# zhaozijie2022/LocoTouch

Hardware: AMD Instinct MI355X
Metric: env-steps/sec (whole node), TransportTeacher 4096 envs/GPU (higher is better)
Workload: dtype f32

## Files before the change

include/lt_env.h:

```cpp
#ifndef LT_ENV_H
#define LT_ENV_H

#include <stddef.h>
#include <stdint.h>

#ifdef __cplusplus
extern "C" {
#endif

#define LT_ABI_VERSION 21

#define LT_OK 0
#define LT_EINVAL (-22)
#define LT_ENOMEM (-12)
#define LT_EFAULT (-14)
#define LT_EHIP (-5)

#define LT_TASK_LOCOMOTION 0
#define LT_TASK_TRANSPORT_TEACHER 1
#define LT_TACTILE_ROWS 17
#define LT_TACTILE_COLS 13
#define LT_TACTILE_DIM 442
#define LT_TACTILE_WIDE_DIM 884
#define LT_TACTILE_BINARY 0
// ... 325 lines not shown
  LT_PRIM_TRUNK = 0, LT_PRIM_BACK_MID = 1, LT_PRIM_PLATE = 2, LT_PRIM_RAIL_LEFT = 3, LT_PRIM_RAIL_RIGHT = 4,
  LT_PRIM_HIP = 5,
  LT_PRIM_THIGH = 9,
  LT_PRIM_CALF = 13,
  LT_PRIM_FOOT = 17,
  LT_PRIM_OBJECT = 21, LT_PRIM_GROUND = 22, LT_RENDER_NUM_PRIMS = 23
};
#define LT_RENDER_MAX_SIZE 8192
#define LT_RENDER_FAR 1000
#define LT_RENDER_DEPTH_MISS 1000000
#define LT_RENDER_VIEWS_PER_LAUNCH 32
typedef struct lt_render_view {
  int32_t env_id;
  int32_t origin;
  float eye[3];
  float lookat[3];
  float fov_y_deg;
} lt_render_view;
typedef struct lt_render_desc {
  int32_t width, height;
  int32_t flags;
  float light_dir[3];
} lt_render_desc;
int lt_env_render(lt_env* env, const lt_render_desc* desc, const lt_render_view* views, int nviews, uint32_t* rgba, float* depth,
                  int32_t* ids, float* poses, void* stream);

const char* lt_env_kernel_name(int which);
enum lt_mlp_mode { LT_MLP_MODE_FORWARD = 0, LT_MLP_MODE_POLICY = 1, LT_MLP_MODE_BACKWARD = 2 };
const char* lt_mlp_kernel_name(const lt_mlp_desc* d0, const lt_mlp_desc* d1_or_null, int64_t m, int mode);

#include "lt_obs_norm.h"
#include "lt_student.h"
#include "lt_collect.h"

#ifdef __cplusplus
}
#endif
#endif
```

locotouch_amd/_abi.py:

```python
from __future__ import annotations

import ctypes
import os
import re

_HERE = os.path.dirname(os.path.abspath(__file__))
REPO = os.path.dirname(_HERE)
HEADER = os.path.join(REPO, "include", "lt_env.h")
OBS_NORM_HEADER = os.path.join(REPO, "include", "lt_obs_norm.h")
STUDENT_HEADER = os.path.join(REPO, "include", "lt_student.h")
COLLECT_HEADER = os.path.join(REPO, "include", "lt_collect.h")
LIB_PATH = os.environ.get("LOCOTOUCH_AMD_LIB", os.path.join(_HERE, "_lib", "liblocotouch_env.so"))

_SCALARS = {"int": ctypes.c_int, "int32_t": ctypes.c_int32, "int64_t": ctypes.c_int64, "uint8_t": ctypes.c_uint8,
            "uint32_t": ctypes.c_uint32, "uint64_t": ctypes.c_uint64, "size_t": ctypes.c_size_t, "float": ctypes.c_float,
            "double": ctypes.c_double}
_DECL = re.compile(r"(?:const\s+)?(\w+)\s*((?:\*\s*(?:const\b\s*)?)*)(\w*)\s*((?:\[[^\]]*\]\s*)*)")


def _ctype(decl, structs, opaque, consts, typed, param):
    m = _DECL.fullmatch(decl.strip())
    if not m:
        return None
    base, stars, name, dims = m.groups()
    depth = stars.count("*")
    try:
        dims = [sum(int(t) if t.strip().isdigit() else consts[t.strip()] for t in d.split("+")) for d in re.findall(r"\[([^\]]*)\]", dims)]
    except KeyError:
        return None
    if param and dims:
        depth, dims = depth + 1, dims[1:]
    t = structs.get(base) or _SCALARS.get(base)
    if (t is None and base not in opaque and base not in ("void", "char")) or depth > 2 or (param and dims):
        return None
    if depth == 0 and t is None:
        return None
    if depth == 1 and base == "char":
        t = ctypes.c_char_p
    elif depth == 1:
        t = ctypes.POINTER(t) if t is not None and (typed or base in structs or base == "size_t") else ctypes.c_void_p
    elif depth == 2:
        t = ctypes.POINTER(ctypes.POINTER(t) if typed and t is not None else ctypes.c_void_p)
    for d in reversed(dims):
        t = t * d
# ... 56 lines not shown
        return {name: py(getattr(self, name)) for name, *_ in self._fields_ if not name.startswith("_")}


CONSTS, STRUCTS, SIGNATURES = parse_header(open(HEADER).read(), bases={"lt_cfg": _CfgMethods})
globals().update(CONSTS)
LtCfg, LtView, LtMlpDesc = STRUCTS["lt_cfg"], STRUCTS["lt_view"], STRUCTS["lt_mlp_desc"]
LtRenderView, LtRenderDesc = STRUCTS["lt_render_view"], STRUCTS["lt_render_desc"]
EXPORTS = list(SIGNATURES)
OBS_NORM_SIGNATURES = parse_header(open(OBS_NORM_HEADER).read())[2]
if any(r is not ctypes.c_int for r, _ in OBS_NORM_SIGNATURES.values()) or set(OBS_NORM_SIGNATURES) & set(EXPORTS):
    raise ImportError("include/lt_obs_norm.h: every entry point returns a status and none repeats one of lt_env.h")

VALUE_QUERIES = frozenset({
    "lt_abi_version", "lt_cfg_sizeof", "lt_cfg_num_presets", "lt_cfg_preset_id", "lt_cfg_obs_dim", "lt_cfg_tactile_dim", "lt_last_error",
    "lt_wgrad_splits", "lt_wgrad_ws_floats", "lt_elu_backward_bias_ws_floats", "lt_head_wgrad_ws_floats", "lt_adam_clip_step_ws_floats",
    "lt_elu_backward_bias_nblk", "lt_head_wgrad_nblk", "lt_mlp_backward_blocks", "lt_env_kernel_name", "lt_mlp_kernel_name"})
if not VALUE_QUERIES <= set(EXPORTS) or any(SIGNATURES[n][0] is not ctypes.c_int for n in set(EXPORTS) - VALUE_QUERIES):
    raise ImportError("_abi.VALUE_QUERIES does not match include/lt_env.h: a query it names is gone, or a new entry point returns no status")

STUDENT_CONSTS, _student_structs, STUDENT_SIGNATURES = parse_header(open(STUDENT_HEADER).read(), structs=STRUCTS)
globals().update(STUDENT_CONSTS)
LtStudentDesc, LtStudentParams = _student_structs["lt_student_desc"], _student_structs["lt_student_params"]
STUDENT_VALUE_QUERIES = frozenset({"lt_student_step_launches"})
if (not STUDENT_VALUE_QUERIES <= set(STUDENT_SIGNATURES) or any(r is not ctypes.c_int for r, _ in STUDENT_SIGNATURES.values())
        or set(STUDENT_SIGNATURES) & (set(EXPORTS) | set(OBS_NORM_SIGNATURES))):
    raise ImportError("_abi.STUDENT_VALUE_QUERIES does not match include/lt_student.h, or an entry point there returns no int or repeats "
                      "one of another header")

COLLECT_SIGNATURES = parse_header(open(COLLECT_HEADER).read())[2]
if (any(r is not ctypes.c_int for r, _ in COLLECT_SIGNATURES.values())
        or set(COLLECT_SIGNATURES) & (set(EXPORTS) | set(OBS_NORM_SIGNATURES) | set(STUDENT_SIGNATURES))):
    raise ImportError("include/lt_collect.h: every entry point returns a status and none repeats one of another header")

_lib = None
_calls: dict = {}


def load() -> ctypes.CDLL:
    global _lib
    if _lib is not None:
        return _lib
    if not os.path.exists(LIB_PATH):
        raise ImportError(f"{LIB_PATH} is missing: run `python -c 'import __graft_entry__ as g; g.build()'` "
                          "(the HIP extension is mandatory, there is no CPU fallback)")
    lib = ctypes.CDLL(LIB_PATH)
    for name, (restype, argtypes) in {**SIGNATURES, **OBS_NORM_SIGNATURES, **STUDENT_SIGNATURES, **COLLECT_SIGNATURES}.items():
        fn = getattr(lib, name)
        fn.restype, fn.argtypes = restype, argtypes
        if name not in VALUE_QUERIES and name not in STUDENT_VALUE_QUERIES:
            _calls[name] = (fn, [ptr if t is ctypes.c_void_p else _ref if issubclass(t, ctypes._Pointer) and issubclass(t._type_, ctypes.Structure)
                                 else None for t in argtypes])
    if lib.lt_cfg_sizeof() != ctypes.sizeof(LtCfg):
        raise ImportError(f"lt_cfg ABI mismatch: C {lib.lt_cfg_sizeof()} vs ctypes {ctypes.sizeof(LtCfg)}")
    if lib.lt_abi_version() != CONSTS["LT_ABI_VERSION"]:
        raise ImportError("lt_env.h / liblocotouch_env.so ABI version mismatch")
    _lib = lib
    return lib


def ptr(x):
    if x is None or isinstance(x, int):
        return ctypes.c_void_p(x or None)
    data_ptr = getattr(x, "data_ptr", None)
    return ctypes.c_void_p(data_ptr()) if data_ptr else x


def _ref(x):
    return ctypes.byref(x) if isinstance(x, ctypes.Structure) else x


def stream(device=None) -> ctypes.c_void_p:
    import torch

    return ctypes.c_void_p(torch.cuda.current_stream(device).cuda_stream)


def ptr_array(tensors):
    return (ctypes.c_void_p * max(1, len(tensors)))(*[None if t is None else t.data_ptr() for t in tensors])

# ... 50 lines not shown
```

locotouch_amd/csrc/lt_ppo.hip:

```cpp
#include <hip/hip_runtime.h>
#include <math.h>
#include <stdint.h>

#include "lt_env.h"
#include "lt_internal.h"

namespace {

constexpr int MAX_A = 16;
constexpr float kHalfLog2Pi = 0.91893853320467274178f;

__global__ __launch_bounds__(256) void lt_ppo_loss_kernel(const float* __restrict__ mu, const float* __restrict__ stdp, const float* __restrict__ value,
                                                          const float* __restrict__ actions, const float* __restrict__ old_logp,
                                                          const float* __restrict__ adv, const float* __restrict__ returns,
                                                          const float* __restrict__ old_values, const float* __restrict__ old_mu,
                                                          const float* __restrict__ old_sigma, const long long* __restrict__ idx,
                                                          long long M, int A, float clip, float vcoef, int clipped_value,
                                                          float* __restrict__ dmu, float* __restrict__ dvalue, float* __restrict__ acc) {
  const long long row = (long long)blockIdx.x * 256 + threadIdx.x;
  const bool ok = row < M;
  const long long src = (ok && idx) ? idx[row] : row;
  float part[4 + MAX_A];
  float amax_mu = 0.f, amax_v = 0.f;
#pragma unroll
// ... 59 lines not shown
    if (lane == 0) red[wave][i] = v;
  }
#pragma unroll
  for (int off = 32; off > 0; off >>= 1) {
    amax_mu = fmaxf(amax_mu, __shfl_xor(amax_mu, off, 64));
    amax_v = fmaxf(amax_v, __shfl_xor(amax_v, off, 64));
  }
  __shared__ float redm[4][2];
  if (lane == 0) { redm[wave][0] = amax_mu; redm[wave][1] = amax_v; }
  __syncthreads();
  if (threadIdx.x < 4 + A && threadIdx.x != 3) {
    const int i = threadIdx.x;
    atomicAdd(acc + i, red[0][i] + red[1][i] + red[2][i] + red[3][i]);
  } else if (threadIdx.x >= 64 && threadIdx.x < 66) {
    const int j = threadIdx.x - 64;
    atomicMax((unsigned*)acc + 20 + j, __float_as_uint(fmaxf(fmaxf(redm[0][j], redm[1][j]), fmaxf(redm[2][j], redm[3][j]))));
  }
}

__global__ __launch_bounds__(64) void lt_ppo_finalize_kernel(const float* __restrict__ acc, const float* __restrict__ stdp, int A, float inv_m,
                                                             float vcoef, float ecoef, float* __restrict__ out) {
  const int a = threadIdx.x;
  float e = 0.f;
  if (a < A) {
    const float sg = stdp[a];
    e = 0.5f + kHalfLog2Pi + logf(sg);
    out[8 + a] = acc[4 + a] - ecoef / sg;
  }
  for (int off = 32; off > 0; off >>= 1) e += __shfl_xor(e, off, 64);
  if (a == 0) {
    const float surr = acc[0] * inv_m, vl = acc[1] * inv_m;
    out[0] = surr + vcoef * vl - ecoef * e;
    out[1] = surr; out[2] = vl; out[3] = e; out[4] = acc[2] * inv_m;
  }
}

constexpr int EB_ROWS = 48;

__global__ __launch_bounds__(256) void lt_elu_bwd_bias_kernel(const float* da, const float* __restrict__ a, long long M, int N, float alpha,
                                                              float* dz, float* __restrict__ ws, float* __restrict__ amax) {
  const int n4 = N >> 2, lanes = 256 / n4;
  const int c4 = threadIdx.x % n4, rl = threadIdx.x / n4;
  const long long r0 = (long long)blockIdx.x * EB_ROWS;
  float4 sum = {0.f, 0.f, 0.f, 0.f};
  float mx = 0.f;
  if (rl < lanes) {
    for (int r = rl; r < EB_ROWS; r += lanes) {
      const long long row = r0 + r;
      if (row >= M) break;
      const float4 g = ((const float4*)(da + row * N))[c4], y = ((const float4*)(a + row * N))[c4];
      float4 o;
      o.x = g.x * (y.x > 0.f ? 1.f : y.x + alpha);
      o.y = g.y * (y.y > 0.f ? 1.f : y.y + alpha);
      o.z = g.z * (y.z > 0.f ? 1.f : y.z + alpha);
      o.w = g.w * (y.w > 0.f ? 1.f : y.w + alpha);
      ((float4*)(dz + row * N))[c4] = o;
      sum.x += o.x; sum.y += o.y; sum.z += o.z; sum.w += o.w;
      mx = fmaxf(fmaxf(mx, fmaxf(fabsf(o.x), fabsf(o.y))), fmaxf(fabsf(o.z), fabsf(o.w)));
    }
  }
  __shared__ float4 red[256];
  __shared__ float redm[4];
  red[threadIdx.x] = sum;
  if (amax) {
#pragma unroll
    for (int off = 32; off > 0; off >>= 1) mx = fmaxf(mx, __shfl_xor(mx, off, 64));
// ... 76 lines not shown
        s[u].x += v.x; s[u].y += v.y; s[u].z += v.z; s[u].w += v.w;
      }
    }
#pragma unroll
    for (int u = 0; u < 3; ++u) {
      if (b < nblk) {
        const float4 v = at(b);
        s[u].x += v.x; s[u].y += v.y; s[u].z += v.z; s[u].w += v.w;
        b += RL;
      }
    }
  }
  __shared__ float4 red[256];
  red[threadIdx.x] = make_float4((s[0].x + s[1].x) + (s[2].x + s[3].x), (s[0].y + s[1].y) + (s[2].y + s[3].y),
                                 (s[0].z + s[1].z) + (s[2].z + s[3].z), (s[0].w + s[1].w) + (s[2].w + s[3].w));
  __syncthreads();
  if (lane == 0 && e < count) {
    float4 t = red[c];
    for (int l = 1; l < RL; ++l) { const float4 v = red[l * cols + c]; t.x += v.x; t.y += v.y; t.z += v.z; t.w += v.w; }
    const float o[4] = {t.x, t.y, t.z, t.w};
#pragma unroll
    for (int i = 0; i < 4; ++i) {
      const int ei = e + i;
      if (ei >= count) break;
      if (ei < split) J.out0[j][ei] = o[i];
      else if (J.out1[j]) J.out1[j][ei - split] = o[i];
    }
  }
}

constexpr int HW_ROWS = 96, HW_MAX_N = 16;

template <int NN>
__global__ __launch_bounds__(256) void lt_head_wgrad_kernel(const float* __restrict__ dy, const float* __restrict__ x, int x_split, long long M, int n, int k,
                                                            float* __restrict__ ws) {
  const int k4 = k >> 2, lanes = 256 / k4;
  const int c4 = threadIdx.x % k4, rl = threadIdx.x / k4;
  const long long r0 = (long long)blockIdx.x * HW_ROWS;
  float4 acc[NN];
  float accb[NN];
#pragma unroll
  for (int j = 0; j < NN; ++j) { acc[j] = {0.f, 0.f, 0.f, 0.f}; accb[j] = 0.f; }
  if (rl < lanes) {
    for (int r = rl; r < HW_ROWS; r += 4 * lanes) {
      float4 xv[4];
      float d[4][NN];
#pragma unroll
      for (int u = 0; u < 4; ++u) {
        const long long row = r0 + r + u * lanes;
        const bool ok = (r + u * lanes) < HW_ROWS && row < M;
        xv[u] = ok ? ((const float4*)(x + row * k))[c4] : float4{0.f, 0.f, 0.f, 0.f};
        if (x_split) {
          const unsigned w[4] = {__float_as_uint(xv[u].x), __float_as_uint(xv[u].y), __float_as_uint(xv[u].z), __float_as_uint(xv[u].w)};
          float f[4];
#pragma unroll
          for (int i = 0; i < 4; ++i)
            f[i] = (float)__builtin_bit_cast(_Float16, (unsigned short)(w[i] & 0xFFFFu)) + (float)__builtin_bit_cast(_Float16, (unsigned short)(w[i] >> 16)) * (1.f / 64.f);
          xv[u] = float4{f[0], f[1], f[2], f[3]};
        }
#pragma unroll
        for (int j = 0; j < NN; ++j) d[u][j] = (ok && j < n) ? dy[row * n + j] : 0.f;
      }
#pragma unroll
      for (int u = 0; u < 4; ++u)
#pragma unroll
        for (int j = 0; j < NN; ++j) {
          acc[j].x += d[u][j] * xv[u].x; acc[j].y += d[u][j] * xv[u].y; acc[j].z += d[u][j] * xv[u].z; acc[j].w += d[u][j] * xv[u].w;
          accb[j] += d[u][j];
        }
    }
  }
  extern __shared__ float4 red[];
  float* const redb = (float*)(red + (size_t)lanes * NN * k4);
  if (rl < lanes) {
#pragma unroll
    for (int j = 0; j < NN; ++j) red[((size_t)rl * NN + j) * k4 + c4] = acc[j];
    if (c4 == 0)
#pragma unroll
      for (int j = 0; j < NN; ++j) redb[rl * NN + j] = accb[j];
  }
  __syncthreads();
  float* const out = ws + (size_t)blockIdx.x * ((size_t)n * k + HW_MAX_N);
  for (int e = threadIdx.x; e < n * k4; e += 256) {
    const int j = e / k4, c = e - j * k4;
    float4 t = red[(size_t)j * k4 + c];
    for (int l = 1; l < lanes; ++l) {
      const float4 u = red[((size_t)l * NN + j) * k4 + c];
      t.x += u.x; t.y += u.y; t.z += u.z; t.w += u.w;
    }
    ((float4*)(out + (size_t)j * k))[c] = t;
  }
  if (threadIdx.x < n) {
    float t = redb[threadIdx.x];
    for (int l = 1; l < lanes; ++l) t += redb[l * NN + threadIdx.x];
    out[(size_t)n * k + threadIdx.x] = t;
  }
}

__global__ __launch_bounds__(256) void lt_gae_kernel(const float* __restrict__ rewards, const unsigned char* __restrict__ dones,
                                                     const float* __restrict__ values, const float* __restrict__ last_values, float gamma,
                                                     float lam, int T, long long N, float* __restrict__ returns, float* __restrict__ advantages) {
  const long long e = (long long)blockIdx.x * 256 + threadIdx.x;
  if (e >= N) return;
  float next_v = last_values[e], gae = 0.f;
  for (int t = T - 1; t >= 0; --t) {
    const long long o = (long long)t * N + e;
    const float v = values[o], alive = 1.f - (float)dones[o];
    const float delta = rewards[o] + alive * gamma * next_v - v;
    gae = delta + alive * gamma * lam * gae;
    const float ret = gae + v;
    returns[o] = ret;
    advantages[o] = ret - v;
    next_v = v;
  }
}

constexpr int AD_PER_BLOCK = 2048;

__global__ __launch_bounds__(256) void lt_sumsq_kernel(const float* __restrict__ g, long long n, float* __restrict__ ws) {
  const long long base = (long long)blockIdx.x * AD_PER_BLOCK;
  float s = 0.f;
  for (int k = threadIdx.x; k < AD_PER_BLOCK; k += 256) {
    const long long i = base + k;
    if (i < n) s += g[i] * g[i];
  }
  for (int off = 32; off > 0; off >>= 1) s += __shfl_xor(s, off, 64);
  __shared__ float red[4];
  if ((threadIdx.x & 63) == 0) red[threadIdx.x >> 6] = s;
  __syncthreads();
// ... 177 lines not shown
    lt_set_error("lt_adam_clip_step: invalid argument");
    return LT_EINVAL;
  }
  const int nblk = (int)((n + AD_PER_BLOCK - 1) / AD_PER_BLOCK);
  const double bc1 = 1.0 - pow((double)beta1, (double)step), bc2 = 1.0 - pow((double)beta2, (double)step);
  hipLaunchKernelGGL(lt_sumsq_kernel, dim3((unsigned)nblk), dim3(256), 0, (hipStream_t)stream, grads, (long long)n, ws);
  hipLaunchKernelGGL(lt_adam_kernel, dim3((unsigned)nblk), dim3(256), 0, (hipStream_t)stream, params, grads, exp_avg, exp_avg_sq, (long long)n, ws, nblk,
                     max_norm, beta1, beta2, eps, weight_decay, (float)((double)lr / bc1), (float)sqrt(bc2), grad_norm, lr_dev, (float)(1.0 / bc1));
  const hipError_t e = hipGetLastError();
  if (e != hipSuccess) { lt_set_error(hipGetErrorString(e)); return LT_EHIP; }
  return LT_OK;
}

extern "C" int64_t lt_adam_clip_step_ws_floats(int64_t n) { return (n + AD_PER_BLOCK - 1) / AD_PER_BLOCK; }

extern "C" int lt_ppo_loss(const float* mu, const float* stdp, const float* value, const float* actions, const float* old_logp, const float* adv,
                           const float* returns, const float* old_values, const float* old_mu, const float* old_sigma, const int64_t* idx,
                           int64_t M, int A, float clip, float value_loss_coef, float entropy_coef, int use_clipped_value_loss, float* dmu, float* dvalue,
                           float* acc, float* out, void* stream) {
  if (!mu || !stdp || !value || !actions || !old_logp || !adv || !returns || !old_values || !old_mu || !old_sigma || !dmu || !dvalue || !acc ||
      M < 1 || A < 1 || A > MAX_A) {
    lt_set_error("lt_ppo_loss: invalid argument (1 <= num_actions <= 16)");
    return LT_EINVAL;
  }
  hipError_t e = hipMemsetAsync(acc, 0, sizeof(float) * (4 + MAX_A + 4), (hipStream_t)stream);
  if (e != hipSuccess) { lt_set_error(hipGetErrorString(e)); return LT_EHIP; }
  hipLaunchKernelGGL(lt_ppo_loss_kernel, dim3((unsigned)((M + 255) / 256)), dim3(256), 0, (hipStream_t)stream, mu, stdp, value, actions, old_logp, adv,
                     returns, old_values, old_mu, old_sigma, (const long long*)idx, (long long)M, A, clip, value_loss_coef, use_clipped_value_loss, dmu, dvalue, acc);
  if (out) hipLaunchKernelGGL(lt_ppo_finalize_kernel, dim3(1), dim3(64), 0, (hipStream_t)stream, acc, stdp, A, 1.f / (float)M, value_loss_coef, entropy_coef, out);
  e = hipGetLastError();
  if (e != hipSuccess) { lt_set_error(hipGetErrorString(e)); return LT_EHIP; }
  return LT_OK;
}
```

locotouch_amd/rl/mlp.py:

```python
from __future__ import annotations

import ctypes
import os

import torch
import torch.nn as nn

from .. import _abi

USE_FUSED_BACKWARD = os.environ.get("LT_FUSED_BACKWARD", "1") != "0"
_ACT_IDS = {nn.ELU: "LT_ACT_ELU", nn.ReLU: "LT_ACT_RELU", nn.Tanh: "LT_ACT_TANH", nn.Identity: "LT_ACT_NONE"}


def describe(seq: nn.Sequential):
    linears, acts = [], set()
    mods = list(seq)
    for i, m in enumerate(mods):
        if isinstance(m, nn.Linear):
            if m.bias is None or m.weight.dtype != torch.float32:
                return None
            linears.append(m)
        elif type(m) in _ACT_IDS:
            if type(m) is nn.ELU and (m.alpha != 1.0):
                return None
            if i == 0 or not isinstance(mods[i - 1], nn.Linear) or i == len(mods) - 1:
                return None
            acts.add(type(m))
        else:
            return None
    C = _abi.CONSTS
    if not linears or len(linears) > C["LT_MLP_MAX_LAYERS"] or len(acts) > 1:
        return None
    if len(linears) > 1 and len(mods) != 2 * len(linears) - 1:
        return None
    dims = [linears[0].in_features] + [l.out_features for l in linears]
    if dims[0] > C["LT_MLP_MAX_WIDTH"] or any(d > 512 for d in dims[1:]):
        return None
    if any(a.out_features != b.in_features for a, b in zip(linears[:-1], linears[1:])):
        return None
    desc = _abi.LtMlpDesc()
    desc.num_layers = len(linears)
    for i, d in enumerate(dims):
        desc.dims[i] = d
# ... 233 lines not shown
        self.domain_max = None
        return v >= float(_abi.CONSTS["LT_MLP_INPUT_CLAMP"])

    def forward_raw(self, x0: torch.Tensor, x1: torch.Tensor, split: bool | None = None):
        if split is None:
            split = self._fused_backward_possible(x0, x1)
        self.acts_split = bool(split)
        self.pack_training(with_backward=self.acts_split)
        ys, acts = _forward_pair((self.a, self.b), x0, x1, self.acts_split)
        if self.check_domain:
            hidden = [t.view(torch.float16)[:, 0::2] if self.acts_split else t for t in (*acts[0], *acts[1])]
            self._record_domain((x0, x1, *hidden))
        return ys, acts

    def pack_training(self, with_backward: bool) -> None:
        args = []
        for net in (self.a, self.b):
            if with_backward:
                net.alloc_bpacked()
            args += [net.desc, net.weight_ptrs(), net.bias_ptrs(), net.packed, net.bpacked if with_backward else None]
        _abi.call("lt_mlp_pack_training", *args, _abi.stream())
        self._bpacked_fresh = bool(with_backward)

    def split_rows(self, x: torch.Tensor) -> torch.Tensor:
        k = x.shape[1]
        if k % 4:
            xp = torch.zeros(x.shape[0], k + (-k) % 4, device=x.device, dtype=torch.float32)
            xp[:, :k] = x
            x = xp
        out = torch.empty_like(x, dtype=torch.float32)
        _abi.call("lt_split_rows", x, out, x.numel(), _abi.stream())
        return out

    def _fused_backward_possible(self, x0, x1) -> bool:
        from .linear import _head_wgrad_ok

        if not USE_FUSED_BACKWARD:
            return False
        if x0.dtype != torch.float32 or x1.dtype != torch.float32 or not x0.is_contiguous() or not x1.is_contiguous():
            return False
        if self._bwd_shapes_ok is None:
            ok = self.a.backward_ok() and self.b.backward_ok()
            for net in (self.a, self.b):
                dims = [net.desc.dims[i] for i in range(net.desc.num_layers + 1)]
                ok = ok and dims[0] % 2 == 0
                ok = ok and _head_wgrad_ok(torch.empty(0, dims[-1], device=x0.device), torch.empty(0, dims[-2], device=x0.device))
            self._bwd_shapes_ok = bool(ok)
        return self._bwd_shapes_ok

    def _fused_backward_ok(self, x0, x1, dy0, dy1) -> bool:
        return self._fused_backward_possible(x0, x1) and dy0.dtype == torch.float32 and dy1.dtype == torch.float32

    def _backward_fused(self, x0, x1, acts, dy0, dy1, grad_of, sums, x_split_rows=None, after_first=None, dy_amax=None) -> None:
        lib = _abi.load()
        stream = _abi.stream()
        m = x0.shape[0]
        nets, xs = (self.a, self.b), (x0, x1)
        asp = int(self.acts_split)
        xsp = int(x_split_rows is not None)
        if not xsp and any(x.shape[1] % 4 for x in xs):
            x_split_rows, xsp = (self.split_rows(x0), self.split_rows(x1)), 1
        if xsp:
            xs = x_split_rows
        dys = [d if d.is_contiguous() else d.contiguous() for d in (dy0, dy1)]
        dev = x0.device
        if self.sat is None:
            self.sat = torch.zeros(1, device=dev, dtype=torch.float32)
        nblk = lib.lt_mlp_backward_blocks(ctypes.byref(nets[0].desc), ctypes.byref(nets[1].desc), m)
        dzs, amaxs, arrs = [], [], []
        per_net = (SumJobs(), SumJobs()) if after_first is not None else (sums, sums)
        for k, net in enumerate(nets):
            if not self._bpacked_fresh:
                net.pack_backward()
            L = len(net.linears)
            n, kk = dys[k].shape[1], acts[k][L - 2].shape[1]
            ws = torch.empty(lib.lt_head_wgrad_ws_floats(m, n, kk), device=dev, dtype=torch.float32)
            _abi.call("lt_head_wgrad", dys[k], acts[k][L - 2], asp, m, n, kk, None, None, ws, stream)
            per_net[k].add(ws, lib.lt_head_wgrad_nblk(m), n * kk + 16, n * kk + n, n * kk, grad_of[net.linears[L - 1].weight], grad_of[net.linears[L - 1].bias])
            dz = [torch.empty_like(a) for a in acts[k]]
            am = torch.empty(L - 1, nblk, device=dev, dtype=torch.float32)
            dzs.append(dz)
            amaxs.append(am)
            arrs.append((_abi.ptr_array(acts[k]), _abi.ptr_array(dz), _abi.ptr_array([am[l] for l in range(L - 1)])))
        dzsp = int(dy_amax is not None)
        scales = torch.empty(2, device=dev, dtype=torch.float32)
        in_amax = dy_amax if dzsp else (None, None)
        _abi.call("lt_mlp_backward_pair", nets[0].desc, nets[0].bpacked, dys[0], *arrs[0], nets[1].desc, nets[1].bpacked, dys[1], *arrs[1],
                  m, asp, in_amax[0], in_amax[1], dzsp, scales, self.sat, stream)
        for k, net in enumerate(nets):
            for l in range(len(net.linears) - 2, -1, -1):
                inp = acts[k][l - 1] if l > 0 else xs[k]
                dz = dzs[k][l]
                n, kk = dz.shape[1], inp.shape[1]
                sp = lib.lt_wgrad_splits(m, n, kk)
                slabs = torch.empty(sp * n * kk + sp * n, device=dev, dtype=torch.float32)
                dbs = slabs[sp * n * kk:]
                _abi.call("lt_wgrad", dz, dzsp, scales[k:k + 1], inp, asp if l > 0 else xsp, m, n, kk, amaxs[k][l], nblk, slabs, dbs, stream)
                gw = grad_of[net.linears[l].weight]
                if kk != gw.shape[1]:
                    pad = torch.empty(n, kk, device=dev, dtype=torch.float32)
                    per_net[k].add(slabs, sp, n * kk, n * kk, n * kk, pad)
                    per_net[k].after.append((gw, pad[:, :gw.shape[1]]))
                else:
                    per_net[k].add(slabs, sp, n * kk, n * kk, n * kk, gw)
                per_net[k].add(dbs, sp, n, n, n, grad_of[net.linears[l].bias])
            if after_first is not None:
                per_net[k].launch()
                if k == 0:
                    after_first()
        self._keep_bwd = (dzs, amaxs, dys, per_net, scales if dzsp else None)
        self._bpacked_fresh = False
# ... 27 lines not shown
```

locotouch_amd/rl/ppo.py:

```python
from __future__ import annotations

import torch
import torch.nn as nn

from .. import _abi
from .dist import Dist
from .modules import ActorCritic
from .storage import RolloutStorage


class PPO:
    def __init__(self, actor_critic: ActorCritic, num_learning_epochs=1, num_mini_batches=1, clip_param=0.2, gamma=0.998,
                 lam=0.95, value_loss_coef=1.0, entropy_coef=0.0, learning_rate=1e-3, max_grad_norm=1.0,
                 use_clipped_value_loss=True, schedule="fixed", desired_kl=0.01, device="cpu",
                 normalize_advantage_per_mini_batch=False, dist: Dist | None = None, **unused):
        self.device = device
        self.dist = dist or Dist()
        self.actor_critic = actor_critic.to(device)
        on_gpu = torch.device(device).type == "cuda"
        self.fused_loss = on_gpu and bool(unused.get("fused_loss", True))
        self.packed_forward = on_gpu and bool(unused.get("packed_forward", True))
        self.direct_update = on_gpu and bool(unused.get("direct_update", True))
        self._pair = None
        if on_gpu and bool(unused.get("tuned_gemms", True)):
            from . import tuned_gemms

            tuned_gemms.enable()
        self.optimizer = torch.optim.Adam(self.actor_critic.parameters(), lr=learning_rate)
        self.storage: RolloutStorage | None = None
        self.learning_rate = learning_rate
        self.schedule, self.desired_kl = schedule, desired_kl
        self.clip_param, self.gamma, self.lam = clip_param, gamma, lam
        self.num_learning_epochs, self.num_mini_batches = num_learning_epochs, num_mini_batches
        self.value_loss_coef, self.entropy_coef, self.max_grad_norm = value_loss_coef, entropy_coef, max_grad_norm
        self.use_clipped_value_loss = use_clipped_value_loss
        self.normalize_advantage_per_mini_batch = normalize_advantage_per_mini_batch
        self._t = {}
        self._flat_grad: torch.Tensor | None = None
        self._flat_adam = None
        use_flat_adam = on_gpu and bool(unused.get("fused_adam", True))
        if self.dist.world_size > 1:
            if not use_flat_adam:
                self._make_flat_grad_bucket()
            self.broadcast_parameters()
        if use_flat_adam:
            from .flat_adam import FlatAdam

            self._flat_adam = FlatAdam(self.optimizer)
            self._flat_grad = self._flat_adam.flat_g

    def _make_flat_grad_bucket(self) -> None:
        params = [p for p in self.actor_critic.parameters() if p.requires_grad]
        total = sum(p.numel() for p in params)
        self._flat_grad = torch.zeros(total, device=params[0].device, dtype=params[0].dtype)
        off = 0
        for p in params:
# ... 91 lines not shown
                mu, ac.std, value, *small, self.clip_param, self.value_loss_coef, self.entropy_coef,
                self.use_clipped_value_loss, idx=idx)
            kl_handle = self.dist.all_reduce_mean_begin(kl_mean.detach().clone()) if adaptive else None
            self._zero_grad()
            loss.backward()
            if adaptive:
                self._apply_kl(self.dist.all_reduce_mean_end(kl_handle), reduced=True)
            self._optim_step()
            stats = stats + torch.stack((value_loss, surrogate_loss, ent.detach()))
        n = self.num_learning_epochs * self.num_mini_batches
        sv, ss, se = (stats / n).tolist()
        if pair is not None and pair.domain_violated():
            self._warn_mlp_domain()
        st.clear()
        return sv, ss, se, None, None

    def _direct_update(self, pair, split_buckets: bool = True):
        ac, st, fa = self.actor_critic, self.storage, self._flat_adam
        obs, cobs, small = self._flat_storage()
        small = [t.view(-1) if t.shape[-1] == 1 else t for t in small]
        dev = obs.device
        adaptive = self.desired_kl is not None and self.schedule == "adaptive"
        a_dim = small[0].shape[1]
        state = torch.zeros(4, device=dev)
        state[0] = self.learning_rate
        lr_dev, stats = state[:1], state[1:]
        grad_of = fa.grad_views()
        std_c = ac.std.detach()
        pair.arm_domain_check()
        n_steps = 0
        critic_at = fa.offset_of(next(iter(ac.critic.parameters())))
        two_buckets = split_buckets and 0 < critic_at < self._flat_grad.numel()
        perm, m = st.mini_batch_permutation(self.num_mini_batches)
        perm_o, perm_co = obs[perm], cobs[perm]
        if perm_o.dtype != torch.float32:
            perm_o, perm_co = perm_o.float(), perm_co.float()
        split_o = (pair.split_rows(perm_o), pair.split_rows(perm_co)) if pair._fused_backward_possible(perm_o[:m], perm_co[:m]) else None
        for step_i in range(self.num_learning_epochs * self.num_mini_batches):
            i = step_i % self.num_mini_batches
            idx = perm[i * m:(i + 1) * m]
            o, co = perm_o[i * m:(i + 1) * m], perm_co[i * m:(i + 1) * m]
            xs = (split_o[0][i * m:(i + 1) * m], split_o[1][i * m:(i + 1) * m]) if split_o is not None else None
            (mu, value), acts = pair.forward_raw(o, co)
            dmu = torch.empty_like(mu)
            dvalue = torch.empty(m, 1, device=dev, dtype=torch.float32)
            acc = torch.empty(24, device=dev, dtype=torch.float32)
            out = torch.empty(24, device=dev, dtype=torch.float32)
            stream = _abi.stream(dev)
            _abi.call("lt_ppo_loss", mu, std_c, value, *small, idx, m, a_dim, float(self.clip_param), float(self.value_loss_coef),
                      float(self.entropy_coef), int(bool(self.use_clipped_value_loss)), dmu, dvalue, acc, out, stream)
            kl = None
            if adaptive:
                kl = out[4:5]
                if self.dist.world_size > 1:
                    kl = self.dist.all_reduce_mean_(kl.clone())
            _abi.call("lt_ppo_lr_rule", kl, float(self.desired_kl or 0.0), 1e-5, 1e-2, 1.5, lr_dev, stats, out, grad_of[ac.std], a_dim, stream)
            if self.dist.world_size > 1 and two_buckets:
                handles = []
                pair.backward_raw(o, co, acts, dmu, dvalue, grad_of, xs, after_first=lambda: handles.append(self.dist.all_reduce_mean_begin(self._flat_grad[:critic_at])),
                                  dy_amax=(acc[20:21], acc[21:22]))
                handles.append(self.dist.all_reduce_mean_begin(self._flat_grad[critic_at:] if handles else self._flat_grad))
                for h in handles:
                    self.dist.all_reduce_mean_end(h)
            else:
                pair.backward_raw(o, co, acts, dmu, dvalue, grad_of, xs, dy_amax=(acc[20:21], acc[21:22]))
                if self.dist.world_size > 1:
                    self.dist.all_reduce_mean_(self._flat_grad)
            fa.step_dev(self.max_grad_norm, lr_dev)
            n_steps += 1
        sat = pair.saturated()
        lr, sv, ss, se, nsat = torch.cat((state, sat if sat is not None else state[:0].new_zeros(1))).tolist()
        if nsat > 0:
            import warnings

            sat.zero_()
            warnings.warn(f"lt_mlp_backward_pair: {int(nsat)} workgroup-layers of the gradient chain reached the f16 image's bound "
                          "(a gradient grew by more than 500x through the layers): those rows were saturated; set LT_FUSED_BACKWARD=0 "
                          "to run the chain as f32 library GEMMs")
        self.learning_rate = lr
        for group in self.optimizer.param_groups:
            group["lr"] = lr
        if pair.domain_violated():
            self._warn_mlp_domain()
        st.clear()
        return sv / n_steps, ss / n_steps, se / n_steps, None, None

    def _warn_mlp_domain(self) -> None:
        import warnings

# ... 113 lines not shown
```

Before: 68.31 million.

## Fuse PPO update launches: loss+lr rule, paired head wgrad, gather+split rows

Several small PPO-update kernels are merged. The loss kernel now also does the finalize and adaptive-LR step through a last-block ticket. The two head weight-gradient launches are combined into one 2D grid, and the minibatch row gather, f32 conversion and hi/lo split are done in one kernel. Per-step scratch buffers are reused across minibatches to cut allocator and launch overhead. This adds an atomic ticket pattern that depends on the acc buffer being zeroed and reset correctly, and the update phase is probably a small share of env-steps/sec.

```diff
diff --git a/include/lt_env.h b/include/lt_env.h
--- a/include/lt_env.h
+++ b/include/lt_env.h
@@ -381,6 +381,7 @@
 #include "lt_obs_norm.h"
 #include "lt_student.h"
 #include "lt_collect.h"
+#include "lt_update.h"
 
 #ifdef __cplusplus
 }
diff --git a/include/lt_update.h b/include/lt_update.h
--- /dev/null
+++ b/include/lt_update.h
@@ -0,0 +1,26 @@
+#ifndef LT_UPDATE_H
+#define LT_UPDATE_H
+
+#include <stdint.h>
+
+#ifdef __cplusplus
+extern "C" {
+#endif
+
+int lt_ppo_loss_step(const float* mu, const float* std, const float* value, const float* actions, const float* old_logp, const float* adv,
+                     const float* returns, const float* old_values, const float* old_mu, const float* old_sigma, const int64_t* idx, int64_t M,
+                     int A, float clip, float value_loss_coef, float entropy_coef, int use_clipped_value_loss, float* dmu, float* dvalue,
+                     float* acc, float* out, float desired_kl, float lr_min, float lr_max, float factor, float* lr, float* stats,
+                     float* dstd_out, void* stream);
+
+int lt_head_wgrad_pair(const float* dy0, const float* x0, int n0, float* ws0, const float* dy1, const float* x1, int n1, float* ws1,
+                       int x_split, int64_t M, int k, void* stream);
+
+int lt_gather_split_rows(const void* src, int src_bf16, const int64_t* perm, int64_t rows, int64_t src_rows, int width, float* out_f32,
+                         void* out_split, void* stream);
+
+#ifdef __cplusplus
+}
+#endif
+
+#endif
diff --git a/locotouch_amd/_abi.py b/locotouch_amd/_abi.py
--- a/locotouch_amd/_abi.py
+++ b/locotouch_amd/_abi.py
@@ -10,6 +10,7 @@
 OBS_NORM_HEADER = os.path.join(REPO, "include", "lt_obs_norm.h")
 STUDENT_HEADER = os.path.join(REPO, "include", "lt_student.h")
 COLLECT_HEADER = os.path.join(REPO, "include", "lt_collect.h")
+UPDATE_HEADER = os.path.join(REPO, "include", "lt_update.h")
 LIB_PATH = os.environ.get("LOCOTOUCH_AMD_LIB", os.path.join(_HERE, "_lib", "liblocotouch_env.so"))
 
 _SCALARS = {"int": ctypes.c_int, "int32_t": ctypes.c_int32, "int64_t": ctypes.c_int64, "uint8_t": ctypes.c_uint8,
@@ -132,6 +133,11 @@
         or set(COLLECT_SIGNATURES) & (set(EXPORTS) | set(OBS_NORM_SIGNATURES) | set(STUDENT_SIGNATURES))):
     raise ImportError("include/lt_collect.h: every entry point returns a status and none repeats one of another header")
 
+UPDATE_SIGNATURES = parse_header(open(UPDATE_HEADER).read())[2]
+if (any(r is not ctypes.c_int for r, _ in UPDATE_SIGNATURES.values())
+        or set(UPDATE_SIGNATURES) & (set(EXPORTS) | set(OBS_NORM_SIGNATURES) | set(STUDENT_SIGNATURES) | set(COLLECT_SIGNATURES))):
+    raise ImportError("include/lt_update.h: every entry point returns a status and none repeats one of another header")
+
 _lib = None
 _calls: dict = {}
 
@@ -144,7 +150,7 @@
         raise ImportError(f"{LIB_PATH} is missing: run `python -c 'import __graft_entry__ as g; g.build()'` "
                           "(the HIP extension is mandatory, there is no CPU fallback)")
     lib = ctypes.CDLL(LIB_PATH)
-    for name, (restype, argtypes) in {**SIGNATURES, **OBS_NORM_SIGNATURES, **STUDENT_SIGNATURES, **COLLECT_SIGNATURES}.items():
+    for name, (restype, argtypes) in {**SIGNATURES, **OBS_NORM_SIGNATURES, **STUDENT_SIGNATURES, **COLLECT_SIGNATURES, **UPDATE_SIGNATURES}.items():
         fn = getattr(lib, name)
         fn.restype, fn.argtypes = restype, argtypes
         if name not in VALUE_QUERIES and name not in STUDENT_VALUE_QUERIES:
diff --git a/locotouch_amd/csrc/lt_ppo.hip b/locotouch_amd/csrc/lt_ppo.hip
--- a/locotouch_amd/csrc/lt_ppo.hip
+++ b/locotouch_amd/csrc/lt_ppo.hip
@@ -115,6 +115,199 @@
     const float surr = acc[0] * inv_m, vl = acc[1] * inv_m;
     out[0] = surr + vcoef * vl - ecoef * e;
     out[1] = surr; out[2] = vl; out[3] = e; out[4] = acc[2] * inv_m;
+  }
+}
+
+constexpr int LS_LANES = 16, LS_ROWS = 256 / LS_LANES, LS_MAX_BLOCKS = 512;
+static_assert(LS_LANES >= MAX_A && 4 + MAX_A <= 20, "a lane per component; lanes 20 .. 23 of the tail own the maxima");
+
+struct LossStepTail {
+  float inv_m, vcoef, ecoef, desired, lr_min, lr_max, factor;
+  float *out, *lr, *stats, *dstd;
+};
+
+__global__ __launch_bounds__(256) void lt_ppo_loss_step_kernel(const float* __restrict__ mu, const float* __restrict__ stdp, const float* __restrict__ value,
+                                                               const float* __restrict__ actions, const float* __restrict__ old_logp,
+                                                               const float* __restrict__ adv, const float* __restrict__ returns,
+                                                               const float* __restrict__ old_values, const float* __restrict__ old_mu,
+                                                               const float* __restrict__ old_sigma, const long long* __restrict__ idx,
+                                                               long long M, int A, float clip, float vcoef, int clipped_value,
+                                                               float* __restrict__ dmu, float* __restrict__ dvalue, float* acc, const LossStepTail T) {
+  const int lane = threadIdx.x & 63, wave = threadIdx.x >> 6;
+  const int sub = lane & (LS_LANES - 1), gbase = lane & ~(LS_LANES - 1);
+  const int grp = threadIdx.x / LS_LANES;
+  const bool comp = sub < A;
+  const float inv_m = 1.f / (float)M;
+  const float sg = comp ? stdp[sub] : 1.f;
+  const float isg = 1.f / sg;
+  float s_surr = 0.f, s_vl = 0.f, s_kl = 0.f, s_dsig = 0.f, amax_mu = 0.f, amax_v = 0.f;
+  for (long long r0 = (long long)blockIdx.x * LS_ROWS; r0 < M; r0 += (long long)gridDim.x * LS_ROWS) {
+    const long long row = r0 + grp;
+    const bool ok = row < M;
+    const long long src = ok ? (idx ? idx[row] : row) : 0;
+    float m = 0.f, x = 0.f, om = 0.f, os = 1.f, advr = 0.f, olp = 0.f, v = 0.f, R = 0.f, ov = 0.f;
+    if (ok) {
+      if (comp) { m = mu[row * A + sub]; x = actions[src * A + sub]; om = old_mu[src * A + sub]; os = old_sigma[src * A + sub]; }
+      advr = adv[src]; olp = old_logp[src]; v = value[row]; R = returns[src];
+      if (clipped_value) ov = old_values[src];
+    }
+    const float z = (x - m) * isg;
+    const float t_logp = -0.5f * z * z - __logf(sg) - kHalfLog2Pi;
+    const float t_kl = __logf(sg / os + 1.0e-5f) + (os * os + (om - m) * (om - m)) / (2.f * sg * sg) - 0.5f;
+    float logp = 0.f, kl = 0.f;
+#pragma unroll
+    for (int a = 0; a < MAX_A; ++a) {
+      if (a < A) {
+        logp += __shfl(t_logp, gbase + a, 64);
+        kl += __shfl(t_kl, gbase + a, 64);
+      }
+    }
+    const float ratio = __expf(logp - olp);
+    const float s1 = -advr * ratio;
+    const float rc = fminf(fmaxf(ratio, 1.f - clip), 1.f + clip);
+    const float s2 = -advr * rc;
+    const bool inside = ratio >= 1.f - clip && ratio <= 1.f + clip;
+    const float dsurr_dratio = (s1 > s2 || inside) ? -advr : 0.f;
+    const float dlogp = dsurr_dratio * ratio * inv_m;
+    if (ok && comp) {
+      dmu[row * A + sub] = dlogp * z * isg;
+      amax_mu = fmaxf(amax_mu, fabsf(dlogp * z * isg));
+      s_dsig += dlogp * (z * z - 1.f) * isg;
+    }
+    float vl, dv;
+    if (clipped_value) {
+      const float dcl = fminf(fmaxf(v - ov, -clip), clip);
+      const float vc = ov + dcl;
+      const float l1 = (v - R) * (v - R), l2 = (vc - R) * (vc - R);
+      const bool in_v = (v - ov) >= -clip && (v - ov) <= clip;
+      vl = fmaxf(l1, l2);
+      dv = (l1 > l2 || in_v) ? 2.f * (v - R) : 0.f;
+    } else {
+      vl = (R - v) * (R - v);
+      dv = 2.f * (v - R);
+    }
+    if (ok && sub == 0) {
+      dvalue[row] = vcoef * dv * inv_m;
+      amax_v = fmaxf(amax_v, fabsf(vcoef * dv * inv_m));
+      s_surr += fmaxf(s1, s2);
+      s_vl += vl;
+      s_kl += kl;
+    }
+  }
+#pragma unroll
+  for (int off = LS_LANES; off < 64; off <<= 1) {
+    s_surr += __shfl_xor(s_surr, off, 64);
+    s_vl += __shfl_xor(s_vl, off, 64);
+    s_kl += __shfl_xor(s_kl, off, 64);
+    s_dsig += __shfl_xor(s_dsig, off, 64);
+    amax_v = fmaxf(amax_v, __shfl_xor(amax_v, off, 64));
+  }
+#pragma unroll
+  for (int off = 32; off > 0; off >>= 1) amax_mu = fmaxf(amax_mu, __shfl_xor(amax_mu, off, 64));
+  __shared__ float red[4][4 + MAX_A];
+  __shared__ float redm[4][2];
+  if (lane < LS_LANES) red[wave][4 + lane] = s_dsig;
+  if (lane == 0) { red[wave][0] = s_surr; red[wave][1] = s_vl; red[wave][2] = s_kl; redm[wave][0] = amax_mu; redm[wave][1] = amax_v; }
+  __syncthreads();
+  if (wave != 0) return;
+  if (lane < 4 + A && lane != 3) {
+    atomicAdd(acc + lane, red[0][lane] + red[1][lane] + red[2][lane] + red[3][lane]);
+  } else if (lane >= 20 && lane < 22) {
+    const int j = lane - 20;
+    atomicMax((unsigned*)acc + 22 + j, __float_as_uint(fmaxf(fmaxf(redm[0][j], redm[1][j]), fmaxf(redm[2][j], redm[3][j]))));
+  }
+  __threadfence();
+  unsigned ticket = 0;
+  if (lane == 0) ticket = atomicAdd((unsigned*)acc + 3, 1u);
+  ticket = __shfl(ticket, 0, 64);
+  if (ticket != gridDim.x - 1) return;
+  float got = 0.f;
+  if (lane < 20) got = __uint_as_float(atomicExch((unsigned*)acc + lane, 0u));
+  else if (lane < 22) got = __uint_as_float(atomicExch((unsigned*)acc + lane + 2, 0u));
+  if (lane >= 20 && lane < 22) acc[lane] = got;
+  const float dsig_sum = __shfl(got, 4 + (lane < MAX_A ? lane : 0), 64);
+  const float sum_surr = __shfl(got, 0, 64), sum_vl = __shfl(got, 1, 64), sum_kl = __shfl(got, 2, 64);
+  float e = 0.f;
+  if (lane < A) {
+    const float s = stdp[lane];
+    e = 0.5f + kHalfLog2Pi + logf(s);
+    const float dsig = dsig_sum - T.ecoef / s;
+    T.out[8 + lane] = dsig;
+    if (T.lr && T.dstd) T.dstd[lane] = dsig;
+  }
+  for (int off = 32; off > 0; off >>= 1) e += __shfl_xor(e, off, 64);
+  if (lane != 0) return;
+  const float surr = sum_surr * T.inv_m, vl = sum_vl * T.inv_m, kl = sum_kl * T.inv_m;
+  T.out[0] = surr + T.vcoef * vl - T.ecoef * e;
+  T.out[1] = surr; T.out[2] = vl; T.out[3] = e; T.out[4] = kl;
+  if (!T.lr) return;
+  if (T.desired > 0.f) {
+    float r = *T.lr;
+    if (kl > T.desired * 2.f) r = fmaxf(T.lr_min, r / T.factor);
+    else if (kl < T.desired * 0.5f && kl > 0.f) r = fminf(T.lr_max, r * T.factor);
+    *T.lr = r;
+  }
+  if (T.stats) { T.stats[0] += vl; T.stats[1] += surr; T.stats[2] += e; }
+}
+
+constexpr int GS_ROWS = 8;
+
+__device__ __forceinline__ unsigned split_word(float x) {
+  const float c = __builtin_amdgcn_fmed3f(x, -(float)LT_MLP_INPUT_CLAMP, (float)LT_MLP_INPUT_CLAMP);
+  const _Float16 h = (_Float16)c;
+  const _Float16 l = (_Float16)((c - (float)h) * 64.f);
+  return (unsigned)__builtin_bit_cast(unsigned short, h) | ((unsigned)__builtin_bit_cast(unsigned short, l) << 16);
+}
+
+template <bool BF16>
+__global__ __launch_bounds__(256) void lt_gather_split_rows_kernel(const void* __restrict__ src, const long long* __restrict__ perm, long long rows,
+                                                                   long long src_rows, int width, float* __restrict__ out_f32,
+                                                                   unsigned* __restrict__ out_split) {
+  const int q = (width + 3) >> 2, w4 = q << 2;
+  const bool vec = (width & 3) == 0;
+  const long long r0 = (long long)blockIdx.x * GS_ROWS;
+  for (int e = threadIdx.x; e < GS_ROWS * q; e += 256) {
+    const int r = e / q, c = (e - r * q) << 2;
+    const long long row = r0 + r;
+    if (row >= rows) break;
+    const long long p = perm[row];
+    float v[4] = {0.f, 0.f, 0.f, 0.f};
+    if (p >= 0 && p < src_rows) {
+      if (BF16) {
+        const unsigned short* s = (const unsigned short*)src + p * width + c;
+        if (vec) {
+          const uint2 w = *(const uint2*)s;
+          v[0] = __uint_as_float(w.x << 16); v[1] = __uint_as_float(w.x & 0xFFFF0000u);
+          v[2] = __uint_as_float(w.y << 16); v[3] = __uint_as_float(w.y & 0xFFFF0000u);
+        } else {
+#pragma unroll
+          for (int i = 0; i < 4; ++i)
+            if (c + i < width) v[i] = __uint_as_float((unsigned)s[i] << 16);
+        }
+      } else {
+        const float* s = (const float*)src + p * width + c;
+        if (vec) {
+          const float4 w = *(const float4*)s;
+          v[0] = w.x; v[1] = w.y; v[2] = w.z; v[3] = w.w;
+        } else {
+#pragma unroll
+          for (int i = 0; i < 4; ++i)
+            if (c + i < width) v[i] = s[i];
+        }
+      }
+    }
+    if (out_f32) {
+      float* o = out_f32 + row * width + c;
+      if (vec) *(float4*)o = make_float4(v[0], v[1], v[2], v[3]);
+      else {
+#pragma unroll
+        for (int i = 0; i < 4; ++i)
+          if (c + i < width) o[i] = v[i];
+      }
+    }
+    if (out_split) {
+      *(uint4*)(out_split + row * w4 + c) = make_uint4(split_word(v[0]), split_word(v[1]), split_word(v[2]), split_word(v[3]));
+    }
   }
 }
 
@@ -257,8 +450,8 @@
 constexpr int HW_ROWS = 96, HW_MAX_N = 16;
 
 template <int NN>
-__global__ __launch_bounds__(256) void lt_head_wgrad_kernel(const float* __restrict__ dy, const float* __restrict__ x, int x_split, long long M, int n, int k,
-                                                            float* __restrict__ ws) {
+__device__ __forceinline__ void head_wgrad_block(const float* __restrict__ dy, const float* __restrict__ x, int x_split, long long M, int n, int k,
+                                                 float* __restrict__ ws, float4* red) {
   const int k4 = k >> 2, lanes = 256 / k4;
   const int c4 = threadIdx.x % k4, rl = threadIdx.x / k4;
   const long long r0 = (long long)blockIdx.x * HW_ROWS;
@@ -295,7 +488,6 @@
         }
     }
   }
-  extern __shared__ float4 red[];
   float* const redb = (float*)(red + (size_t)lanes * NN * k4);
   if (rl < lanes) {
 #pragma unroll
@@ -320,6 +512,22 @@
     for (int l = 1; l < lanes; ++l) t += redb[l * NN + threadIdx.x];
     out[(size_t)n * k + threadIdx.x] = t;
   }
+}
+
+template <int NN>
+__global__ __launch_bounds__(256) void lt_head_wgrad_kernel(const float* __restrict__ dy, const float* __restrict__ x, int x_split, long long M, int n, int k,
+                                                            float* __restrict__ ws) {
+  extern __shared__ float4 head_red[];
+  head_wgrad_block<NN>(dy, x, x_split, M, n, k, ws, head_red);
+}
+
+template <int NN0>
+__global__ __launch_bounds__(256) void lt_head_wgrad_pair_kernel(const float* __restrict__ dy0, const float* __restrict__ x0, int n0, float* __restrict__ ws0,
+                                                                 const float* __restrict__ dy1, const float* __restrict__ x1, float* __restrict__ ws1,
+                                                                 int x_split, long long M, int k) {
+  extern __shared__ float4 head_red[];
+  if (blockIdx.y == 0) head_wgrad_block<NN0>(dy0, x0, x_split, M, n0, k, ws0, head_red);
+  else head_wgrad_block<1>(dy1, x1, x_split, M, 1, k, ws1, head_red);
 }
 
 __global__ __launch_bounds__(256) void lt_gae_kernel(const float* __restrict__ rewards, const unsigned char* __restrict__ dones,
@@ -563,3 +771,79 @@
   if (e != hipSuccess) { lt_set_error(hipGetErrorString(e)); return LT_EHIP; }
   return LT_OK;
 }
+
+extern "C" int lt_ppo_loss_step(const float* mu, const float* stdp, const float* value, const float* actions, const float* old_logp, const float* adv,
+                                const float* returns, const float* old_values, const float* old_mu, const float* old_sigma, const int64_t* idx,
+                                int64_t M, int A, float clip, float value_loss_coef, float entropy_coef, int use_clipped_value_loss, float* dmu,
+                                float* dvalue, float* acc, float* out, float desired_kl, float lr_min, float lr_max, float factor, float* lr,
+                                float* stats, float* dstd_out, void* stream) {
+  if (!mu || !stdp || !value || !actions || !old_logp || !adv || !returns || !old_values || !old_mu || !old_sigma || !dmu || !dvalue || !acc ||
+      !out || M < 1 || A < 1 || A > MAX_A || (lr && factor <= 1.f)) {
+    lt_set_error("lt_ppo_loss_step: invalid argument (1 <= num_actions <= 16, out required, factor > 1 with a learning rate)");
+    return LT_EINVAL;
+  }
+  LossStepTail T;
+  T.inv_m = 1.f / (float)M; T.vcoef = value_loss_coef; T.ecoef = entropy_coef;
+  T.desired = desired_kl; T.lr_min = lr_min; T.lr_max = lr_max; T.factor = factor;
+  T.out = out; T.lr = lr; T.stats = stats; T.dstd = dstd_out;
+  const int64_t want = (M + LS_ROWS - 1) / LS_ROWS;
+  const unsigned blocks = (unsigned)(want < LS_MAX_BLOCKS ? want : LS_MAX_BLOCKS);
+  hipLaunchKernelGGL(lt_ppo_loss_step_kernel, dim3(blocks), dim3(256), 0, (hipStream_t)stream, mu, stdp, value, actions, old_logp, adv, returns,
+                     old_values, old_mu, old_sigma, (const long long*)idx, (long long)M, A, clip, value_loss_coef, use_clipped_value_loss, dmu, dvalue,
+                     acc, T);
+  const hipError_t e = hipGetLastError();
+  if (e != hipSuccess) { lt_set_error(hipGetErrorString(e)); return LT_EHIP; }
+  return LT_OK;
+}
+
+extern "C" int lt_head_wgrad_pair(const float* dy0, const float* x0, int n0, float* ws0, const float* dy1, const float* x1, int n1, float* ws1,
+                                  int x_split, int64_t M, int k, void* stream) {
+  if (!dy0 || !x0 || !ws0 || !dy1 || !x1 || !ws1 || M < 1 || n0 < 1 || n0 > HW_MAX_N || n1 != 1 || k < 4 || (k & 3) || k > 1024) {
+    lt_set_error("lt_head_wgrad_pair: invalid argument (1 <= n0 <= 16, n1 == 1, k a multiple of 4, 4 <= k <= 1024)");
+    return LT_EINVAL;
+  }
+  const int nblk = (int)((M + HW_ROWS - 1) / HW_ROWS), k4 = k / 4, lanes = 256 / k4;
+  const int nn = n0 <= 1 ? 1 : (n0 <= 4 ? 4 : (n0 <= 8 ? 8 : (n0 <= 12 ? 12 : 16)));
+  const size_t lds = (size_t)lanes * nn * k4 * 16 + (size_t)lanes * nn * 4;
+  if (const int e = lt_ensure_dynamic_lds((const void*)lt_head_wgrad_pair_kernel<16>, 72 * 1024)) {
+    lt_set_error(hipGetErrorString((hipError_t)e));
+    return LT_EHIP;
+  }
+  if (lds > 72 * 1024) {
+    lt_set_error("lt_head_wgrad_pair: n0 * k too large for one block's LDS partials");
+    return LT_EINVAL;
+  }
+  const dim3 g((unsigned)nblk, 2), b(256);
+  hipStream_t st = (hipStream_t)stream;
+  switch (nn) {
+    case 1: hipLaunchKernelGGL(lt_head_wgrad_pair_kernel<1>, g, b, lds, st, dy0, x0, n0, ws0, dy1, x1, ws1, x_split, (long long)M, k); break;
+    case 4: hipLaunchKernelGGL(lt_head_wgrad_pair_kernel<4>, g, b, lds, st, dy0, x0, n0, ws0, dy1, x1, ws1, x_split, (long long)M, k); break;
+    case 8: hipLaunchKernelGGL(lt_head_wgrad_pair_kernel<8>, g, b, lds, st, dy0, x0, n0, ws0, dy1, x1, ws1, x_split, (long long)M, k); break;
+    case 12: hipLaunchKernelGGL(lt_head_wgrad_pair_kernel<12>, g, b, lds, st, dy0, x0, n0, ws0, dy1, x1, ws1, x_split, (long long)M, k); break;
+    default: hipLaunchKernelGGL(lt_head_wgrad_pair_kernel<16>, g, b, lds, st, dy0, x0, n0, ws0, dy1, x1, ws1, x_split, (long long)M, k); break;
+  }
+  const hipError_t e = hipGetLastError();
+  if (e != hipSuccess) { lt_set_error(hipGetErrorString(e)); return LT_EHIP; }
+  return LT_OK;
+}
+
+extern "C" int lt_gather_split_rows(const void* src, int src_bf16, const int64_t* perm, int64_t rows, int64_t src_rows, int width, float* out_f32,
+                                    void* out_split, void* stream) {
+  const bool vec = width > 0 && (width & 3) == 0;
+  const auto misaligned = [](const void* p, uintptr_t a) { return (reinterpret_cast<uintptr_t>(p) & (a - 1)) != 0; };
+  if (!src || !perm || rows < 1 || src_rows < 1 || width < 1 || (!out_f32 && !out_split) || misaligned(out_split, 16) ||
+      (vec && (misaligned(src, src_bf16 ? 8 : 16) || misaligned(out_f32, 16)))) {
+    lt_set_error("lt_gather_split_rows: invalid argument (rows, src_rows, width >= 1; an output; 16-byte aligned operands)");
+    return LT_EINVAL;
+  }
+  const dim3 g((unsigned)((rows + GS_ROWS - 1) / GS_ROWS)), b(256);
+  if (src_bf16)
+    hipLaunchKernelGGL(lt_gather_split_rows_kernel<true>, g, b, 0, (hipStream_t)stream, src, (const long long*)perm, (long long)rows, (long long)src_rows,
+                       width, out_f32, (unsigned*)out_split);
+  else
+    hipLaunchKernelGGL(lt_gather_split_rows_kernel<false>, g, b, 0, (hipStream_t)stream, src, (const long long*)perm, (long long)rows, (long long)src_rows,
+                       width, out_f32, (unsigned*)out_split);
+  const hipError_t e = hipGetLastError();
+  if (e != hipSuccess) { lt_set_error(hipGetErrorString(e)); return LT_EHIP; }
+  return LT_OK;
+}
diff --git a/locotouch_amd/rl/mlp.py b/locotouch_amd/rl/mlp.py
--- a/locotouch_amd/rl/mlp.py
+++ b/locotouch_amd/rl/mlp.py
@@ -9,6 +9,10 @@
 from .. import _abi
 
 USE_FUSED_BACKWARD = os.environ.get("LT_FUSED_BACKWARD", "1") != "0"
+
+
+def legacy_launches() -> bool:
+    return os.environ.get("LT_UPDATE_LEGACY_LAUNCHES", "0") == "1"
 _ACT_IDS = {nn.ELU: "LT_ACT_ELU", nn.ReLU: "LT_ACT_RELU", nn.Tanh: "LT_ACT_TANH", nn.Identity: "LT_ACT_NONE"}
 
 
@@ -308,6 +312,15 @@
         _abi.call("lt_split_rows", x, out, x.numel(), _abi.stream())
         return out
 
+    def gather_split_rows(self, src: torch.Tensor, perm: torch.Tensor, want_split: bool = True):
+        if src.dtype not in (torch.float32, torch.bfloat16) or not src.is_contiguous() or perm.dtype != torch.int64 or not perm.is_contiguous():
+            raise ValueError("gather_split_rows: contiguous f32 / bf16 rows and a contiguous int64 permutation")
+        rows, k = perm.numel(), src.shape[1]
+        out = torch.empty(rows, k, device=src.device, dtype=torch.float32)
+        split = torch.empty(rows, k + (-k) % 4, device=src.device, dtype=torch.float32) if want_split else None
+        _abi.call("lt_gather_split_rows", src, int(src.dtype == torch.bfloat16), perm, rows, src.shape[0], k, out, split, _abi.stream(src.device))
+        return out, split
+
     def _fused_backward_possible(self, x0, x1) -> bool:
         from .linear import _head_wgrad_ok
 
@@ -345,14 +358,23 @@
         nblk = lib.lt_mlp_backward_blocks(ctypes.byref(nets[0].desc), ctypes.byref(nets[1].desc), m)
         dzs, amaxs, arrs = [], [], []
         per_net = (SumJobs(), SumJobs()) if after_first is not None else (sums, sums)
+        heads = []
+        for k, net in enumerate(nets):
+            L = len(net.linears)
+            n, kk = dys[k].shape[1], acts[k][L - 2].shape[1]
+            ws = torch.empty(lib.lt_head_wgrad_ws_floats(m, n, kk), device=dev, dtype=torch.float32)
+            heads.append((dys[k], acts[k][L - 2], n, kk, ws))
+            per_net[k].add(ws, lib.lt_head_wgrad_nblk(m), n * kk + 16, n * kk + n, n * kk, grad_of[net.linears[L - 1].weight], grad_of[net.linears[L - 1].bias])
+        (d0, i0, n0, k0, w0), (d1, i1, n1, k1, w1) = heads
+        if n1 == 1 and k0 == k1 and not legacy_launches():
+            _abi.call("lt_head_wgrad_pair", d0, i0, n0, w0, d1, i1, n1, w1, asp, m, k0, stream)
+        else:
+            for d, i, n, kk, w in heads:
+                _abi.call("lt_head_wgrad", d, i, asp, m, n, kk, None, None, w, stream)
         for k, net in enumerate(nets):
             if not self._bpacked_fresh:
                 net.pack_backward()
             L = len(net.linears)
-            n, kk = dys[k].shape[1], acts[k][L - 2].shape[1]
-            ws = torch.empty(lib.lt_head_wgrad_ws_floats(m, n, kk), device=dev, dtype=torch.float32)
-            _abi.call("lt_head_wgrad", dys[k], acts[k][L - 2], asp, m, n, kk, None, None, ws, stream)
-            per_net[k].add(ws, lib.lt_head_wgrad_nblk(m), n * kk + 16, n * kk + n, n * kk, grad_of[net.linears[L - 1].weight], grad_of[net.linears[L - 1].bias])
             dz = [torch.empty_like(a) for a in acts[k]]
             am = torch.empty(L - 1, nblk, device=dev, dtype=torch.float32)
             dzs.append(dz)
diff --git a/locotouch_amd/rl/ppo.py b/locotouch_amd/rl/ppo.py
--- a/locotouch_amd/rl/ppo.py
+++ b/locotouch_amd/rl/ppo.py
@@ -22,6 +22,7 @@
         self.packed_forward = on_gpu and bool(unused.get("packed_forward", True))
         self.direct_update = on_gpu and bool(unused.get("direct_update", True))
         self._pair = None
+        self._update_scratch = None
         if on_gpu and bool(unused.get("tuned_gemms", True)):
             from . import tuned_gemms
 
@@ -179,29 +180,51 @@
         critic_at = fa.offset_of(next(iter(ac.critic.parameters())))
         two_buckets = split_buckets and 0 < critic_at < self._flat_grad.numel()
         perm, m = st.mini_batch_permutation(self.num_mini_batches)
-        perm_o, perm_co = obs[perm], cobs[perm]
-        if perm_o.dtype != torch.float32:
-            perm_o, perm_co = perm_o.float(), perm_co.float()
-        split_o = (pair.split_rows(perm_o), pair.split_rows(perm_co)) if pair._fused_backward_possible(perm_o[:m], perm_co[:m]) else None
+        from .mlp import legacy_launches
+
+        legacy = legacy_launches()
+        want_split = pair._fused_backward_possible(obs[:1].float(), cobs[:1].float())
+        if legacy or not (obs.is_contiguous() and cobs.is_contiguous() and perm.is_contiguous()):
+            perm_o, perm_co = obs[perm], cobs[perm]
+            if perm_o.dtype != torch.float32:
+                perm_o, perm_co = perm_o.float(), perm_co.float()
+            split_o = (pair.split_rows(perm_o), pair.split_rows(perm_co)) if want_split else None
+        else:
+            (perm_o, so), (perm_co, sco) = pair.gather_split_rows(obs, perm, want_split), pair.gather_split_rows(cobs, perm, want_split)
+            split_o = (so, sco) if want_split else None
+        fold_rule = not legacy and self.dist.world_size == 1
+        if not legacy:
+            buf = self._update_scratch
+            if buf is None or buf[0].shape != (m, a_dim) or buf[0].device != dev:
+                buf = self._update_scratch = tuple(make(shape, device=dev, dtype=torch.float32) for make, shape in
+                                                   ((torch.empty, (m, a_dim)), (torch.empty, (m, 1)), (torch.zeros, 24), (torch.empty, 24)))
+            dmu, dvalue, acc, out = buf
         for step_i in range(self.num_learning_epochs * self.num_mini_batches):
             i = step_i % self.num_mini_batches
             idx = perm[i * m:(i + 1) * m]
             o, co = perm_o[i * m:(i + 1) * m], perm_co[i * m:(i + 1) * m]
             xs = (split_o[0][i * m:(i + 1) * m], split_o[1][i * m:(i + 1) * m]) if split_o is not None else None
             (mu, value), acts = pair.forward_raw(o, co)
-            dmu = torch.empty_like(mu)
-            dvalue = torch.empty(m, 1, device=dev, dtype=torch.float32)
-            acc = torch.empty(24, device=dev, dtype=torch.float32)
-            out = torch.empty(24, device=dev, dtype=torch.float32)
             stream = _abi.stream(dev)
-            _abi.call("lt_ppo_loss", mu, std_c, value, *small, idx, m, a_dim, float(self.clip_param), float(self.value_loss_coef),
-                      float(self.entropy_coef), int(bool(self.use_clipped_value_loss)), dmu, dvalue, acc, out, stream)
+            loss_args = (mu, std_c, value, *small, idx, m, a_dim, float(self.clip_param), float(self.value_loss_coef),
+                         float(self.entropy_coef), int(bool(self.use_clipped_value_loss)))
+            if legacy:
+                dmu = torch.empty_like(mu)
+                dvalue = torch.empty(m, 1, device=dev, dtype=torch.float32)
+                acc = torch.empty(24, device=dev, dtype=torch.float32)
+                out = torch.empty(24, device=dev, dtype=torch.float32)
+                _abi.call("lt_ppo_loss", *loss_args, dmu, dvalue, acc, out, stream)
+            else:
+                rule = (lr_dev, stats, grad_of[ac.std]) if fold_rule else (None, None, None)
+                _abi.call("lt_ppo_loss_step", *loss_args, dmu, dvalue, acc, out, float(self.desired_kl or 0.0) if adaptive else 0.0,
+                          1e-5, 1e-2, 1.5, *rule, stream)
             kl = None
             if adaptive:
                 kl = out[4:5]
                 if self.dist.world_size > 1:
                     kl = self.dist.all_reduce_mean_(kl.clone())
-            _abi.call("lt_ppo_lr_rule", kl, float(self.desired_kl or 0.0), 1e-5, 1e-2, 1.5, lr_dev, stats, out, grad_of[ac.std], a_dim, stream)
+            if not fold_rule:
+                _abi.call("lt_ppo_lr_rule", kl, float(self.desired_kl or 0.0), 1e-5, 1e-2, 1.5, lr_dev, stats, out, grad_of[ac.std], a_dim, stream)
             if self.dist.world_size > 1 and two_buckets:
                 handles = []
                 pair.backward_raw(o, co, acts, dmu, dvalue, grad_of, xs, after_first=lambda: handles.append(self.dist.all_reduce_mean_begin(self._flat_grad[:critic_at])),
```

Result: no change. 68.20 million (median of 2 runs) (-0.2%).
